# vanTeeffelenLab/ExTrack

Hardware: AMD Instinct MI355X
Metric: log-likelihood evals/sec (1e6 tracks, 2-state, len=30) (higher is better)
Workload: dtype f64

## Files before the change

### extrack_amd/csrc/xt_reg2.h

```cpp
#pragma once
#include "xt_fast2.h"
#include "xt_grad.h"


template <int F>
struct XtR2Geom {
    static constexpr int NGB = F - 1;
    static constexpr int NG = 1 << NGB;
    static constexpr int TPW = 64 / NG;
};
XT_HD constexpr int xt_r2_gbit(int F, int i) { return F == 7 ? i : (i < 2 ? i : i + 1); }
XT_HD constexpr int xt_r2_gmask(int F) { return F == 7 ? 63 : (F == 6 ? 0x3b : (F == 5 ? 0x1b : 0x0b)); }
template <int F>
XT_HD int xt_r2_slot(int lane)
{
    if (F == 7) return 0;
    int ts = (lane >> 2) & 1;
    if (F == 5) ts |= ((lane >> 5) & 1) << 1;
    if (F == 4) ts |= ((lane >> 4) & 3) << 1;
    return ts;
}

#define XT_R2_TAN0 XT_F2_TAB_BYTES
#define XT_R2_TB 36
#define XT_R2_MAXU 4
XT_HD int xt_r2_pos0(int NP) { return XT_R2_TAN0 + NP * XT_R2_TB * 8; }
XT_HD int xt_r2_acc0(int NP, int D, int KS, int tpw) { return xt_r2_pos0(NP) + XT_F2_WAVES * tpw * XT_F2_CHUNK * (D + KS) * 8; }
XT_HD int xt_r2_block_bytes(int NP, int D, int KS, int tpw) { return xt_r2_acc0(NP, D, KS, tpw) + XT_F2_WAVES * 8 * (NP + 3) * 8; }
#define XT_R2_TAB0 (XT_BLOB_HDR * 8)
#define XT_R2_GC_OFF 800
#define XT_R2_LNT_OFF 960
#define XT_R2_LNT_REL (XT_R2_LNT_OFF - XT_R2_TAB0)
static_assert(XT_R2_GC_OFF >= (XT_BLOB_HDR + XT_NTAB * 4 + 64) * 8 && XT_R2_GC_OFF + 16 <= XT_F2_NAN_OFF, "g-form constants overlap the blob / the NaN flags");
static_assert(XT_R2_LNT_OFF >= XT_F2_NAN_OFF + XT_F2_WAVES * 8 * 4 && XT_R2_LNT_OFF + 64 <= XT_F2_EXPB_OFF, "lnT' overlaps the NaN flags / the exp table");

static inline bool xt_use_reg2(int S, int NS, int F) { return S == 2 && NS == 1 && F >= 4 && F <= 7; }

template <int D, int K, int NP>
struct XtR2Lane {
    double z[2];
    int e[2];
    double m[2][D], u[2][K];
    double rz[NP ? NP : 1][2], dm[NP ? NP : 1][2][D], du[NP ? NP : 1][2][K];
};

template <int F, int D, int K, int NP, int H, bool ZF, bool LAZY, int VAR, bool FIRST = false, class Ctx>
XT_HD void xt_r2_step(Ctx& cx, char* lds, XtR2Lane<D, K, NP>& s, int tab, const double* c, const double* l2)
{
    static_assert(!FIRST || (NP == 0 && ZF && LAZY), "the merge-free first step is a step of the zero-free likelihood-only loop");
    constexpr int NGB = F - 1;
    constexpr int XB = xt_r2_gbit(F, H), PB = xt_r2_gbit(F, (H + NGB - 1) % NGB);
    const int lane = xt_opaque(cx.lane());
    const int prev = (lane >> PB) & 1;
    const int qa = Ctx::template pair_natural<XB>() ? 0 : (lane >> XB) & 1;
    const int io[2] = {(prev * 2 + qa) * 8, (prev * 2 + (qa ^ 1)) * 8};
    double TT[2], TD2[2];
    XT_UNROLL
    for (int q = 0; q < 2; ++q) {
        TT[q] = xt_at<double>(lds, tab + io[q]);
        TD2[q] = xt_at<double>(lds, XT_R2_TAB0 + 4 * 32 + io[q]);
    }

    const int e0 = s.e[0], e1 = s.e[1];
    const int emax = e0 > e1 ? e0 : e1;
    const double w0 = FIRST ? 1.0 : xt_ldexp(s.z[0], e0 - emax), w1 = FIRST ? 0.0 : xt_ldexp(s.z[1], e1 - emax);
    const double W = FIRST ? 1.0 : w0 + w1;
    double M[D], U[K];
    XT_UNROLL
    for (int d = 0; d < D; ++d) M[d] = FIRST ? s.m[0][d] : xt_fma(w1, s.m[1][d], w0 * s.m[0][d]);
    XT_UNROLL
    for (int k = 0; k < K; ++k) U[k] = FIRST ? s.u[0][k] : xt_fma(w1, s.u[1][k], w0 * s.u[0][k]);
    const bool live = ZF ? true : W > 0.0;
    const double Ws = ZF ? W : (live ? W : 1.0);
    constexpr bool RN = !LAZY || (H % XT_F2_RENORM) == 0;
    const double Wm = FIRST ? s.z[0] : (RN ? xt_frexp_mant(W) : W);
    const int We = FIRST ? e0 : (live ? (RN ? emax + xt_frexp_exp(W) : emax) : XT_EMIN);

    double Dq[2][K];
    XT_UNROLL
    for (int q = 0; q < 2; ++q)
        XT_UNROLL
        for (int k = 0; k < K; ++k) Dq[q][k] = xt_fma(Ws, l2[k] + TD2[q], U[k]);
    double rD[2][K], rW;
    if (K == 1) {
        const double d01 = Dq[0][0] * Dq[1][0];
        const double R = xt_rcp(Ws * d01);
        const double RW = R * Ws;
        rW = FIRST ? 1.0 : R * d01;
        rD[0][0] = RW * Dq[1][0];
        rD[1][0] = RW * Dq[0][0];
    } else {
        double f[2 * K + 1], pre[2 * K + 2], suf[2 * K + 2];
        f[0] = Ws;
        XT_UNROLL
        for (int q = 0; q < 2; ++q)
            XT_UNROLL
            for (int k = 0; k < K; ++k) f[1 + q * K + k] = Dq[q][k];
        pre[0] = 1.0;
        XT_UNROLL
        for (int i = 0; i < 2 * K + 1; ++i) pre[i + 1] = pre[i] * f[i];
        suf[2 * K + 1] = 1.0;
        XT_UNROLL
        for (int i = 2 * K; i >= 0; --i) suf[i] = suf[i + 1] * f[i];
        const double R = xt_rcp(pre[2 * K + 1]);
        rW = FIRST ? 1.0 : R * suf[1];
        XT_UNROLL
        for (int q = 0; q < 2; ++q)
            XT_UNROLL
            for (int k = 0; k < K; ++k) rD[q][k] = R * pre[1 + q * K + k] * suf[2 + q * K + k];
    }
    double dmW[D], dsqW = 0.0;
    XT_UNROLL
    for (int d = 0; d < D; ++d) {
        dmW[d] = xt_fma(c[d], Ws, -M[d]);
        if (K == 1) dsqW = xt_fma(dmW[d], dmW[d], dsqW);
    }
    double x[2], gf[2], tt[2][K];
    const double A = -0.5 * rW * dsqW;
    XT_UNROLL
    for (int q = 0; q < 2; ++q) {
        if (K == 1) {
            x[q] = A * rD[q][0];
            tt[q][0] = xt_fma(Ws, TD2[q], U[0]) * rD[q][0];
            gf[q] = xt_pow_half<D>(Ws * rD[q][0]);
        } else {
            double xx = 0.0, gg = 1.0;
            XT_UNROLL
            for (int d = 0; d < D; ++d) {
                xx = xt_fma(dmW[d] * dmW[d], rD[q][d], xx);
                tt[q][d] = xt_fma(Ws, TD2[q], U[d]) * rD[q][d];
                gg *= Ws * rD[q][d];
            }
            x[q] = xx * (-0.5 * rW);
            gf[q] = sqrt(gg);
        }
    }
    double p[2];
    int j[2], n[2];
    xt_exp_tab_x2(x[0], x[1], p[0], p[1], j[0], j[1], n[0], n[1]);
    double nz[2], nm[2][D], nu[2][K];
    int ne[2];
    XT_UNROLL
    for (int q = 0; q < 2; ++q) {
        int en = We + n[q];
        const double tj = xt_at<double>(lds, XT_F2_EXPB_OFF + j[q] * 8);
        double zn = (Wm * TT[q]) * (gf[q] * tj) * p[q];
        if (!LAZY) {
            en += xt_frexp_exp(zn);
            zn = xt_frexp_mant(zn);
        }
        nz[q] = zn;
        ne[q] = en > XT_EMIN ? en : XT_EMIN;
        XT_UNROLL
        for (int d = 0; d < D; ++d) nm[q][d] = xt_fma(dmW[d], tt[q][K == 1 ? 0 : d], M[d]) * rW;
        XT_UNROLL
        for (int k = 0; k < K; ++k) nu[q][k] = l2[k] * tt[q][k];
    }

    double a0 = 0.0, a1 = 0.0, cm[D], cu[K], dn[D], Aq[2][K], rq[2][K];
    if (NP > 0) {
        a0 = w0 * rW;
        a1 = w1 * rW;
        const double aa = a0 * a1;
        XT_UNROLL
        for (int d = 0; d < D; ++d) {
            cm[d] = aa * (s.m[0][d] - s.m[1][d]);
            dn[d] = dmW[d] * rW;
        }
        XT_UNROLL
        for (int k = 0; k < K; ++k) cu[k] = aa * (s.u[0][k] - s.u[1][k]);
        XT_UNROLL
        for (int q = 0; q < 2; ++q)
            XT_UNROLL
            for (int k = 0; k < K; ++k) {
                rq[q][k] = Ws * rD[q][k];
                if (K == 1)
                    Aq[q][0] = -0.5 * rq[q][0] * xt_fma(-(dsqW * rW * rW), rq[q][0], (double)D);
                else
                    Aq[q][k] = -0.5 * rq[q][k] * xt_fma(-(dn[k] * dn[k]), rq[q][k], 1.0);
            }
    }
    cx.template pair_exchange<XB>(nz[0], nz[1]);
    cx.template pair_exchange_i32<XB>(ne[0], ne[1]);
    XT_UNROLL
    for (int d = 0; d < D; ++d) cx.template pair_exchange<XB>(nm[0][d], nm[1][d]);
    XT_UNROLL
    for (int k = 0; k < K; ++k) cx.template pair_exchange<XB>(nu[0][k], nu[1][k]);
    XT_UNROLL
    for (int q = 0; q < 2; ++q) {
        s.z[q] = nz[q];
        s.e[q] = ne[q];
        XT_UNROLL
        for (int d = 0; d < D; ++d) s.m[q][d] = nm[q][d];
        XT_UNROLL
        for (int k = 0; k < K; ++k) s.u[q][k] = nu[q][k];
    }
    if (NP > 0) {
        XT_UNROLL
        for (int pp = 0; pp < NP; ++pp) {
            if (!(VAR & 1)) xt_sched_fence();
            const int tb = XT_R2_TAN0 + pp * XT_R2_TB * 8;
            double dl[K];
            XT_UNROLL
            for (int k = 0; k < K; ++k) dl[k] = xt_at<double>(lds, tb + k * 8);
            const double del = s.rz[pp][0] - s.rz[pp][1];
            const double R = xt_fma(a0, s.rz[pp][0], a1 * s.rz[pp][1]);
            double dmb[D], dub[K];
            XT_UNROLL
            for (int d = 0; d < D; ++d) dmb[d] = xt_fma(cm[d], del, xt_fma(a0, s.dm[pp][0][d], a1 * s.dm[pp][1][d]));
            XT_UNROLL
            for (int k = 0; k < K; ++k) dub[k] = xt_fma(cu[k], del, xt_fma(a0, s.du[pp][0][k], a1 * s.du[pp][1][k]));
            double hd[K];
            if (K == 1) {
                hd[0] = 0.0;
                XT_UNROLL
                for (int d = 0; d < D; ++d) hd[0] = xt_fma(dn[d], dmb[d], hd[0]);
            } else {
                XT_UNROLL
                for (int d = 0; d < D; ++d) hd[d] = dn[d] * dmb[d];
            }
            double trz[2], tdm[2][D], tdu[2][K];
            XT_UNROLL
            for (int q = 0; q < 2; ++q) {
                const double dlT = xt_at<double>(lds, tb + tab + io[q]);
                const double dd2 = xt_at<double>(lds, tb + XT_R2_TAB0 + 4 * 32 + io[q]);
                double rzn = R + dlT, dtt[K];
                XT_UNROLL
                for (int k = 0; k < K; ++k) {
                    const double ds2 = dd2 + dub[k], dden = dl[k] + ds2;
                    dtt[k] = rq[q][k] * xt_fma(-tt[q][k], dden, ds2);
                    rzn = xt_fma(Aq[q][k], dden, rzn);
                    rzn = xt_fma(rq[q][k], hd[k], rzn);
                    tdu[q][k] = xt_fma(l2[k], dtt[k], dl[k] * tt[q][k]);
                }
                trz[q] = ZF ? rzn : (live ? rzn : 0.0);
                XT_UNROLL
                for (int d = 0; d < D; ++d) {
                    const int kk = K == 1 ? 0 : d;
                    tdm[q][d] = xt_fma(dn[d], dtt[kk], xt_fma(-tt[q][kk], dmb[d], dmb[d]));
                }
            }
            cx.template pair_exchange<XB>(trz[0], trz[1]);
            XT_UNROLL
            for (int d = 0; d < D; ++d) cx.template pair_exchange<XB>(tdm[0][d], tdm[1][d]);
            XT_UNROLL
            for (int k = 0; k < K; ++k) cx.template pair_exchange<XB>(tdu[0][k], tdu[1][k]);
            XT_UNROLL
            for (int q = 0; q < 2; ++q) {
                s.rz[pp][q] = trz[q];
                XT_UNROLL
                for (int d = 0; d < D; ++d) s.dm[pp][q][d] = tdm[q][d];
                XT_UNROLL
                for (int k = 0; k < K; ++k) s.du[pp][q][k] = tdu[q][k];
            }
        }
    }
}

template <int F, int D, int H, bool FIRST = false, class Ctx>
XT_HD void xt_r2_step_g(Ctx& cx, char* lds, XtR2Lane<D, 1, 0>& s, int tab, const double* c)
{
    constexpr int NGB = F - 1;
    constexpr int XB = xt_r2_gbit(F, H), PB = xt_r2_gbit(F, (H + NGB - 1) % NGB);
    const int lane = xt_opaque(cx.lane());
    const int prev = (lane >> PB) & 1;
    const int qa = Ctx::template pair_natural<XB>() ? 0 : (lane >> XB) & 1;
    const int io[2] = {(prev * 2 + qa) * 8, (prev * 2 + (qa ^ 1)) * 8};
    double TD2[2], LT[2];
    XT_UNROLL
    for (int q = 0; q < 2; ++q) {
        TD2[q] = xt_at<double>(lds, XT_R2_TAB0 + 4 * 32 + io[q]);
        LT[q] = xt_at<double>(lds, tab + XT_R2_LNT_REL + io[q]);
    }
    const double l2 = xt_at<double>(lds, 0), nh = xt_at<double>(lds, XT_R2_GC_OFF), l22 = xt_at<double>(lds, XT_R2_GC_OFF + 8);

    const int e0 = s.e[0], e1 = s.e[1];
    const int emax = e0 > e1 ? e0 : e1;
    const double w0 = FIRST ? 1.0 : xt_ldexp(s.z[0], e0 - emax), w1 = FIRST ? 0.0 : xt_ldexp(s.z[1], e1 - emax);
    const double Ws = FIRST ? 1.0 : w0 + w1;
    double M[D];
    XT_UNROLL
    for (int d = 0; d < D; ++d) M[d] = FIRST ? s.m[0][d] : xt_fma(w1, s.m[1][d], w0 * s.m[0][d]);
    const double V = FIRST ? s.u[0][0] : xt_fma(w1, s.u[1][0], w0 * s.u[0][0]);
    constexpr bool RN = (H % XT_F2_RENORM) == 0;
    const double Wm = FIRST ? s.z[0] : (RN ? xt_frexp_mant(Ws) : Ws);
    const int We = FIRST ? e0 : (RN ? emax + xt_frexp_exp(Ws) : emax);

    const double Dq0 = xt_fma(Ws, TD2[0], V), Dq1 = xt_fma(Ws, TD2[1], V);
    const double d01 = Dq0 * Dq1;
    const double R = xt_rcp(Ws * d01);
    const double rW = FIRST ? 1.0 : R * d01;
    const double G = R * (Ws * (Ws * l2));
    const double g[2] = {G * Dq1, G * Dq0};
    double dn[D], dsq = 0.0;
    XT_UNROLL
    for (int d = 0; d < D; ++d) {
        dn[d] = xt_fma(c[d], Ws, -M[d]) * rW;
        dsq = xt_fma(dn[d], dn[d], dsq);
    }
    const double A = dsq * nh;
    double p[2];
    int j[2], n[2];
    xt_exp_tab_x2(xt_fma(A, g[0], LT[0]), xt_fma(A, g[1], LT[1]), p[0], p[1], j[0], j[1], n[0], n[1]);
    double nz[2], nm[2][D], nv[2];
    int ne[2];
    XT_UNROLL
    for (int q = 0; q < 2; ++q) {
        const int en = We + n[q];
        const double tj = xt_at<double>(lds, XT_F2_EXPB_OFF + j[q] * 8);
        nz[q] = (Wm * xt_pow_half<D>(g[q])) * (tj * p[q]);
        ne[q] = en > XT_EMIN ? en : XT_EMIN;
        XT_UNROLL
        for (int d = 0; d < D; ++d) nm[q][d] = xt_fma(-dn[d], g[q], c[d]);
        nv[q] = xt_fma(-l2, g[q], l22);
    }
    cx.template pair_exchange<XB>(nz[0], nz[1]);
    cx.template pair_exchange_i32<XB>(ne[0], ne[1]);
    XT_UNROLL
    for (int d = 0; d < D; ++d) cx.template pair_exchange<XB>(nm[0][d], nm[1][d]);
    cx.template pair_exchange<XB>(nv[0], nv[1]);
    XT_UNROLL
    for (int q = 0; q < 2; ++q) {
        s.z[q] = nz[q];
        s.e[q] = ne[q];
        XT_UNROLL
        for (int d = 0; d < D; ++d) s.m[q][d] = nm[q][d];
        s.u[q][0] = nv[q];
    }
}

template <int F, class Ctx>
XT_HD double xt_r2_gsum(Ctx& cx, double v)
{
    constexpr int NGB = F - 1;
    v += cx.template xor_f64<xt_r2_gbit(F, 0)>(v);
    v += cx.template xor_f64<xt_r2_gbit(F, 1)>(v);
    v += cx.template xor_f64<xt_r2_gbit(F, 2)>(v);
    if (NGB > 3) v += cx.template xor_f64<xt_r2_gbit(F, NGB > 3 ? 3 : 0)>(v);
    if (NGB > 4) v += cx.template xor_f64<xt_r2_gbit(F, NGB > 4 ? 4 : 0)>(v);
    if (NGB > 5) v += cx.template xor_f64<xt_r2_gbit(F, NGB > 5 ? 5 : 0)>(v);
    return v;
}
template <int F, class Ctx>
XT_HD int xt_r2_gmax(Ctx& cx, int v)
{
    constexpr int NGB = F - 1;
    auto mx = [](int a, int b) XT_INL { return a > b ? a : b; };
    v = mx(v, cx.template xor_i32<xt_r2_gbit(F, 0)>(v));
    v = mx(v, cx.template xor_i32<xt_r2_gbit(F, 1)>(v));
    v = mx(v, cx.template xor_i32<xt_r2_gbit(F, 2)>(v));
    if (NGB > 3) v = mx(v, cx.template xor_i32<xt_r2_gbit(F, NGB > 3 ? 3 : 0)>(v));
    if (NGB > 4) v = mx(v, cx.template xor_i32<xt_r2_gbit(F, NGB > 4 ? 4 : 0)>(v));
    if (NGB > 5) v = mx(v, cx.template xor_i32<xt_r2_gbit(F, NGB > 5 ? 5 : 0)>(v));
    return v;
}

template <int F, int D, int K, int NP, class Ctx, class GetPos>
XT_HD void xt_r2_chain(Ctx& cx, char* lds, XtR2Lane<D, K, NP>& s, int T, int stay_from, GetPos& getpos)
{
    constexpr int NGB = F - 1;
    const int lane = xt_opaque(cx.lane());
    double z = s.z[0];
    int e = s.e[0];
    XT_UNROLL
    for (int t = 1; t < NGB; ++t) {
        if (t > T) break;
        const int prev = (lane >> xt_r2_gbit(F, t == 1 ? NGB - 1 : t - 2)) & 1;
        const int q = (lane >> xt_r2_gbit(F, t - 1)) & 1;
        const int io = (prev * 2 + q) * 8;
        const double TT = xt_at<double>(lds, XT_R2_TAB0 + (t >= stay_from ? 32 : 0) + io);
        const double d2 = xt_at<double>(lds, XT_R2_TAB0 + 4 * 32 + io);
        double c[D], l2[K];
        getpos(t, c, l2);
        double tt[K], r[K], dm[D], x = 0.0, gf;
        XT_UNROLL
        for (int k = 0; k < K; ++k) {
            const double a = d2 + s.u[0][k];
            r[k] = xt_rcp(l2[k] + a);
            tt[k] = a * r[k];
        }
        XT_UNROLL
        for (int d = 0; d < D; ++d) dm[d] = c[d] - s.m[0][d];
        if (K == 1) {
            XT_UNROLL
            for (int d = 0; d < D; ++d) x = xt_fma(dm[d], dm[d], x);
            x *= -0.5 * r[0];
            gf = xt_pow_half<D>(r[0]);
        } else {
            double gg = 1.0;
            XT_UNROLL
            for (int d = 0; d < D; ++d) {
                x = xt_fma(-0.5 * dm[d] * dm[d], r[d], x);
                gg *= r[d];
            }
            gf = sqrt(gg);
        }
        double p;
        int j, n;
        xt_exp_tab_x1(x, p, j, n);
        z = (z * TT) * (gf * xt_at<double>(lds, XT_F2_EXPB_OFF + j * 8)) * p;
        e += n;
        XT_UNROLL
        for (int d = 0; d < D; ++d) s.m[0][d] = xt_fma(dm[d], tt[K == 1 ? 0 : d], s.m[0][d]);
        XT_UNROLL
        for (int k = 0; k < K; ++k) s.u[0][k] = l2[k] * tt[k];
    }
    int dummy = 0;
    XT_UNROLL
    for (int i = 0; i < NGB - 1; ++i)
        if (i >= T) dummy |= 1 << xt_r2_gbit(F, i);
    const bool live = (lane & dummy) == 0;
    s.z[0] = live ? xt_frexp_mant(z) : 0.0;
    s.e[0] = live ? e + xt_frexp_exp(z) : XT_EMIN;
}

template <int F, int D, int K, int NP, int VAR = 0, class Ctx>
XT_HD void xt_r2_body(const XtKernelArgs& a, const XtGradArgs& ga, Ctx& cx)
{
    int lb, nb;
    const XtBucketDesc b = xt_bind_bucket(a, cx.block(), cx.nblocks(), lb, nb);
    typedef XtR2Geom<F> Gm;
    constexpr int NGB = Gm::NGB, TPW = Gm::TPW;
    constexpr int GMASK = xt_r2_gmask(F);
    const int lane = cx.lane();
    const int wib = cx.wave_in_block();
    const int nwb = cx.waves_per_block();
    const int L = b.L;
    const int KS = a.locerr_mode ? a.KS : 0;
    double* smem = cx.smem();
    char* lds = (char*)smem;

    const int ntab = xt_tab_doubles(2, 2);
    for (int i = cx.tid(); i < ntab; i += cx.nthreads()) smem[i] = xt_blob_ptr(a)[i];
    if (NP > 0)
        for (int i = cx.tid(); i < NP * XT_R2_TB; i += cx.nthreads()) xt_at<double>(lds, XT_R2_TAN0 + i * 8) = ga.dblob[i];
    const int NU = NP > 0 ? ga.NU : 0, NPT = NP + NU;
    for (int i = cx.tid(); i < NU * XT_R2_TB; i += cx.nthreads()) xt_at<double>(lds, XT_R2_TAN0 + (NP * XT_R2_TB + i) * 8) = ga.udblob[i];
    cx.sync();
    xt_f2_check_lds_base(lds);
    xt_f2_build_exp_table(cx, lds, XT_F2_EXPB_OFF, (const double*)(lds + XT_F2_T64_OFF));
    const bool gform = NP == 0 && K == 1 && a.well_scaled == 2 && a.locerr_mode == 0;
    if constexpr (NP == 0 && K == 1) {
        if (gform && cx.tid() < 10) {
            const int i = cx.tid();
            const double l2 = smem[0];
            if (i < 8)
                xt_at<double>(lds, XT_R2_LNT_OFF + i * 8) = log(smem[XT_BLOB_HDR + i]) - 0.5 * D * log(l2);
            else
                xt_at<double>(lds, XT_R2_GC_OFF + (i - 8) * 8) = i == 8 ? -0.5 / l2 : 2.0 * l2;
        }
    }
    cx.sync();
    const double* hdr = smem;

    const int ts = xt_r2_slot<F>(lane);
    const bool leader = (lane & GMASK) == 0;
    const int tlast = L - 1;
    const int stay_from = a.min_len > 2 ? a.min_len : 2;
    const int vfin = (b.isBL ? 2 : 0) + (tlast >= stay_from ? 1 : 0);
    double l2g[K];
    XT_UNROLL
    for (int k = 0; k < K; ++k) l2g[k] = hdr[k];
    const bool well_scaled = a.well_scaled != 0;
    const bool chain = NP == 0 && well_scaled;

    double* pos = (double*)(lds + xt_r2_pos0(NPT)) + wib * TPW * XT_F2_CHUNK * (D + KS);
    double* sig = pos + TPW * XT_F2_CHUNK * D;
    double* accp = (double*)(lds + xt_r2_acc0(NPT, D, KS, TPW)) + (wib * 8 + ts) * (NPT + 3);
    if (leader) {
        if (NP == 0) {
            accp[0] = 1.0;
            accp[1] = 0.0;
            accp[2] = 0.0;
        } else {
            for (int i = 0; i < NPT + 1; ++i) accp[i] = 0.0;
        }
    }

    const int64_t nbatch = (b.N + TPW - 1) / TPW;
    const int64_t W0 = (int64_t)lb * nwb + wib, NW = (int64_t)nb * nwb;
    for (int64_t batch = W0; batch < nbatch; batch += NW) {
        const int64_t trk = batch * TPW + ts;
        const bool act = trk < b.N;

        auto stage = [&](int p0) XT_INL {
            cx.wave_sync();
            for (int i = lane; i < TPW * XT_F2_CHUNK * D; i += 64) {
                const int t_ = i / (XT_F2_CHUNK * D), r = i - t_ * (XT_F2_CHUNK * D);
                const int64_t tk = batch * TPW + t_;
                const int64_t tkc = tk < b.N ? tk : b.N - 1;
                const int pp = p0 + r / D;
                if (pp < L) {
                    const double v = b.tracks[(tkc * L + p0) * D + r];
                    pos[i] = v;
                    if (v != v) xt_at<int>(lds, XT_F2_NAN_OFF + (wib * 8 + t_) * 4) = 1;
                }
            }
            if (KS)
                for (int i = lane; i < TPW * XT_F2_CHUNK * KS; i += 64) {
                    const int t_ = i / (XT_F2_CHUNK * KS), r = i - t_ * (XT_F2_CHUNK * KS);
                    const int64_t tk = batch * TPW + t_;
                    const int64_t tkc = tk < b.N ? tk : b.N - 1;
                    const int pp = p0 + r / KS;
                    if (pp < L) {
                        const double v = b.sigma[(tkc * L + p0) * KS + r];
                        sig[i] = v;
                        if (v != v) xt_at<int>(lds, XT_F2_NAN_OFF + (wib * 8 + t_) * 4) = 1;
                    }
                }
            cx.wave_sync();
        };
        auto getpos = [&](int t, double* c, double* l2) XT_INL {
            const int r = t & (XT_F2_CHUNK - 1);
            XT_UNROLL
            for (int d = 0; d < D; ++d) c[d] = pos[(ts * XT_F2_CHUNK + r) * D + d];
            if (KS == 0) {
                XT_UNROLL
                for (int k = 0; k < K; ++k) l2[k] = xt_at<double>(lds, k * 8);
            } else {
                XT_UNROLL
                for (int k = 0; k < K; ++k) {
                    double sg = sig[(ts * XT_F2_CHUNK + r) * KS + (KS == 1 ? 0 : k)];
                    if (a.locerr_mode == 2) {
                        sg = xt_fma(sg, hdr[3], hdr[4]);
                        sg = sg < 1e-6 ? 1e-6 : sg;
                    }
                    l2[k] = sg * sg;
                }
            }
        };

        XtR2Lane<D, K, NP> s;
#define XT_R2_PHASE(H, ZF_, LAZY_)                                                                     \
    if (NGB > (H) && t <= tend2 && ph == (H)) {                                                        \
        double c[D], l2[K];                                                                            \
        getpos(t, c, l2);                                                                              \
        xt_r2_step<F, D, K, NP, ((H) < NGB ? (H) : 0), ZF_, LAZY_, VAR>(cx, lds, s, XT_R2_TABSEL, c, l2);   \
        ++t;                                                                                           \
        ph = (H) + 1 == NGB ? 0 : (H) + 1;                                                             \
    }
#define XT_R2_PHASE_G(H)                                                                               \
    if (NGB > (H) && t <= tend2 && ph == (H)) {                                                        \
        double c[D], l2[K];                                                                            \
        getpos(t, c, l2);                                                                              \
        xt_r2_step_g<F, D, ((H) < NGB ? (H) : 0)>(cx, lds, s, XT_R2_TABSEL, c);                        \
        ++t;                                                                                           \
        ph = (H) + 1 == NGB ? 0 : (H) + 1;                                                             \
    }
#define XT_R2_PHASES(ZF_, LAZY_) \
    XT_R2_PHASE(0, ZF_, LAZY_)   \
    XT_R2_PHASE(1, ZF_, LAZY_)   \
    XT_R2_PHASE(2, ZF_, LAZY_)   \
    XT_R2_PHASE(3, ZF_, LAZY_)   \
    XT_R2_PHASE(4, ZF_, LAZY_)   \
    XT_R2_PHASE(5, ZF_, LAZY_)
#define XT_R2_TABSEL tab
        auto run_steps = [&](int& t, int tend, int tab) XT_INL {
            int ph = (t - 1) % NGB;
            const int tend2 = tend;
            if (!well_scaled) {
                while (t <= tend2) { XT_R2_PHASES(false, false) }
                return;
            }
            if constexpr (NP == 0 && K == 1) {
                if (gform) {
                    while (t <= tend2) {
                        XT_R2_PHASE_G(0)
                        XT_R2_PHASE_G(1)
                        XT_R2_PHASE_G(2)
                        XT_R2_PHASE_G(3)
                        XT_R2_PHASE_G(4)
                        XT_R2_PHASE_G(5)
                    }
                    return;
                }
            }
            while (t <= tend2) { XT_R2_PHASES(true, true) }
        };
#undef XT_R2_TABSEL
#define XT_R2_TABSEL (XT_R2_TAB0 + (t >= stay_from ? 32 : 0))
        auto run_steps_g = [&](int& t, int tend) XT_INL {
            int ph = (t - 1) % NGB;
            const int tend2 = tend;
            if (well_scaled) {
                while (t <= tend2) { XT_R2_PHASES(false, true) }
            } else {
                while (t <= tend2) { XT_R2_PHASES(false, false) }
            }
        };
#undef XT_R2_TABSEL
#undef XT_R2_PHASES
#undef XT_R2_PHASE_G
#undef XT_R2_PHASE

        XtAcc tot;
        tot.clear();
        double gacc[NP ? NP : 1];
        double uacc[XT_R2_MAXU];
        int fe = XT_EMIN;
        int t = 1;
        if (lane < 8) xt_at<int>(lds, XT_F2_NAN_OFF + (wib * 8 + lane) * 4) = 0;
        for (int p0 = 0; p0 < L; p0 += XT_F2_CHUNK) {
            stage(p0);
            if (p0 == 0) {
                constexpr int NBIT = xt_r2_gbit(F, NGB - 1);
                double c0[D], l20[K];
                getpos(0, c0, l20);
                const bool live0 = chain || (lane & (GMASK & ~(1 << NBIT))) == 0;
                const int s0 = (lane >> NBIT) & 1;
                s.z[0] = live0 ? hdr[8 + s0] : 0.0;
                s.e[0] = live0 ? 0 : XT_EMIN;
                s.z[1] = 0.0;
                s.e[1] = XT_EMIN;
                XT_UNROLL
                for (int q = 0; q < 2; ++q) {
                    XT_UNROLL
                    for (int d = 0; d < D; ++d) s.m[q][d] = c0[d];
                    XT_UNROLL
                    for (int k = 0; k < K; ++k) s.u[q][k] = l20[k];
                }
                XT_UNROLL
                for (int pp = 0; pp < NP; ++pp) {
                    const int tb = XT_R2_TAN0 + pp * XT_R2_TB * 8;
                    s.rz[pp][0] = live0 ? xt_at<double>(lds, tb + (8 + s0) * 8) : 0.0;
                    s.rz[pp][1] = 0.0;
                    XT_UNROLL
                    for (int q = 0; q < 2; ++q) {
                        XT_UNROLL
                        for (int d = 0; d < D; ++d) s.dm[pp][q][d] = 0.0;
                        XT_UNROLL
                        for (int k = 0; k < K; ++k) s.du[pp][q][k] = xt_at<double>(lds, tb + k * 8);
                    }
                }
                if constexpr (NP == 0) {
                    if (chain) {
                        const int T = L - 2 < NGB - 1 ? L - 2 : NGB - 1;
                        xt_r2_chain<F>(cx, lds, s, T, stay_from, getpos);
                        if (L - 2 >= F - 1) {
                            double c[D], l2[K];
                            getpos(F - 1, c, l2);
                            bool first_done = false;
                            if constexpr (K == 1) {
                                if (gform) {
                                    s.u[0][0] += l2[0];
                                    xt_r2_step_g<F, D, NGB - 1, true>(cx, lds, s, XT_R2_TAB0 + (F - 1 >= stay_from ? 32 : 0), c);
                                    first_done = true;
                                }
                            }
                            if (!first_done) xt_r2_step<F, D, K, NP, NGB - 1, true, true, VAR, true>(cx, lds, s, XT_R2_TAB0 + (F - 1 >= stay_from ? 32 : 0), c, l2);
                            t = F;
                        } else {
                            t = L - 1 > 1 ? L - 1 : 1;
                        }
                    }
                }
            }
            const int tend = (L - 2 < p0 + XT_F2_CHUNK - 1) ? L - 2 : p0 + XT_F2_CHUNK - 1;
            if (NP == 0) {
                run_steps(t, tend < stay_from - 1 ? tend : stay_from - 1, XT_R2_TAB0);
                run_steps(t, tend, XT_R2_TAB0 + 32);
            } else {
                run_steps_g(t, tend);
            }
            if (tlast < p0 || tlast >= p0 + XT_F2_CHUNK) continue;
            double cl[D], l2l[K];
            getpos(tlast, cl, l2l);
            if constexpr (NP == 0 && K == 1) {
                if (gform && L - 2 >= F - 1) l2l[0] = 0.0;
            }
            const int hp = (tlast - 2 + NGB) % NGB;
            const int pbit = (F == 7 || hp < 2) ? hp : hp + 1;
            const int prev = (lane >> pbit) & 1;
            double wm[4], rr[4][K], dq[2][D], dsqQ[2];
            int we[4];
            XT_UNROLL
            for (int Q = 0; Q < 2; ++Q) {
                dsqQ[Q] = 0.0;
                XT_UNROLL
                for (int d = 0; d < D; ++d) {
                    dq[Q][d] = cl[d] - s.m[Q][d];
                    dsqQ[Q] = xt_fma(dq[Q][d], dq[Q][d], dsqQ[Q]);
                }
                double x[2], gf[2];
                XT_UNROLL
                for (int q = 0; q < 2; ++q) {
                    const double d2 = xt_at<double>(lds, XT_R2_TAB0 + 4 * 32 + (prev * 2 + q) * 8);
                    if (K == 1) {
                        const double r = xt_rcp(d2 + s.u[Q][0] + l2l[0]);
                        rr[Q * 2 + q][0] = r;
                        x[q] = -0.5 * dsqQ[Q] * r;
                        gf[q] = xt_pow_half<D>(r);
                    } else {
                        double xx = 0.0, gg = 1.0;
                        XT_UNROLL
                        for (int d = 0; d < D; ++d) {
                            const double r = xt_rcp(d2 + s.u[Q][d] + l2l[d]);
                            rr[Q * 2 + q][d] = r;
                            xx = xt_fma(-0.5 * dq[Q][d] * dq[Q][d], r, xx);
                            gg *= r;
                        }
                        x[q] = xx;
                        gf[q] = sqrt(gg);
                    }
                }
                double p[2];
                int j[2], n[2];
                xt_exp_tab_x2(x[0], x[1], p[0], p[1], j[0], j[1], n[0], n[1]);
                XT_UNROLL
                for (int q = 0; q < 2; ++q) {
                    const double tf = xt_at<double>(lds, XT_R2_TAB0 + vfin * 32 + (prev * 2 + q) * 8);
                    wm[Q * 2 + q] = s.z[Q] * tf * gf[q] * xt_at<double>(lds, XT_F2_EXPB_OFF + j[q] * 8) * p[q];
                    we[Q * 2 + q] = s.e[Q] + n[q];
                    tot.add(wm[Q * 2 + q], we[Q * 2 + q]);
                }
            }
            fe = xt_r2_gmax<F>(cx, tot.m != 0.0 ? tot.e : XT_EMIN);
            if (NP > 0) {
                double ws[4];
                XT_UNROLL
                for (int i = 0; i < 4; ++i) ws[i] = wm[i] != 0.0 ? xt_ldexp(wm[i], we[i] - fe) : 0.0;
                XT_UNROLL
                for (int pp = 0; pp < NP; ++pp) {
                    const int tb = XT_R2_TAN0 + pp * XT_R2_TB * 8;
                    double dl[K];
                    XT_UNROLL
                    for (int k = 0; k < K; ++k) dl[k] = xt_at<double>(lds, tb + k * 8);
                    double acc = 0.0;
                    XT_UNROLL
                    for (int Q = 0; Q < 2; ++Q) {
                        XT_UNROLL
                        for (int q = 0; q < 2; ++q) {
                            const double dlT = xt_at<double>(lds, tb + XT_R2_TAB0 + vfin * 32 + (prev * 2 + q) * 8);
                            const double dd2 = xt_at<double>(lds, tb + XT_R2_TAB0 + 4 * 32 + (prev * 2 + q) * 8);
                            double rel = s.rz[pp][Q] + dlT;
                            if (K == 1) {
                                const double r = rr[Q * 2 + q][0];
                                const double dden = dd2 + s.du[pp][Q][0] + dl[0];
                                double ddsq = 0.0;
                                XT_UNROLL
                                for (int d = 0; d < D; ++d) ddsq = xt_fma(-2.0 * dq[Q][d], s.dm[pp][Q][d], ddsq);
                                rel -= 0.5 * r * (D * dden + ddsq - dsqQ[Q] * r * dden);
                            } else {
                                XT_UNROLL
                                for (int d = 0; d < D; ++d) {
                                    const double r = rr[Q * 2 + q][d];
                                    const double dden = dd2 + s.du[pp][Q][d] + dl[d];
                                    rel -= 0.5 * r * (dden - 2.0 * dq[Q][d] * s.dm[pp][Q][d] - dq[Q][d] * dq[Q][d] * r * dden);
                                }
                            }
                            acc = xt_fma(ws[Q * 2 + q], ws[Q * 2 + q] != 0.0 ? rel : 0.0, acc);
                        }
                    }
                    gacc[pp] = acc;
                }
                XT_UNROLL
                for (int u = 0; u < XT_R2_MAXU; ++u) {
                    double acc = 0.0;
                    if (u < NU) {
                        const int tb = XT_R2_TAN0 + (NP + u) * XT_R2_TB * 8;
                        XT_UNROLL
                        for (int i = 0; i < 4; ++i) acc = xt_fma(ws[i], xt_at<double>(lds, tb + XT_R2_TAB0 + vfin * 32 + (prev * 2 + (i & 1)) * 8), acc);
                    }
                    uacc[u] = acc;
                }
            }
        }
        double sum = xt_r2_gsum<F>(cx, tot.m != 0.0 ? xt_ldexp(tot.m, tot.e - fe) : 0.0);
        const bool poisoned = xt_at<int>(lds, XT_F2_NAN_OFF + (wib * 8 + ts) * 4) != 0;
        if (poisoned) sum = NAN;
        if (NP == 0) {
            if (act && leader) {
                if (b.ll_out) b.ll_out[trk] = log(sum) + (double)fe * XT_LN2 + b.ll_const;
                const double pm = accp[0] * xt_frexp_mant(sum);
                double acce = accp[1] + (double)(fe + xt_frexp_exp(sum) + xt_frexp_exp(pm));
                if (sum == 0.0) acce = -INFINITY;
                accp[0] = xt_frexp_mant(pm);
                accp[1] = acce;
                accp[2] += 1.0;
            }
        } else {
            const double rs = 1.0 / sum;
            double gsum[NP ? NP : 1];
            XT_UNROLL
            for (int pp = 0; pp < NP; ++pp) gsum[pp] = xt_r2_gsum<F>(cx, gacc[pp]);
            double usum[XT_R2_MAXU];
            XT_UNROLL
            for (int u = 0; u < XT_R2_MAXU; ++u) usum[u] = u < NU ? xt_r2_gsum<F>(cx, uacc[u]) : 0.0;
            if (act && leader) {
                const double ll = log(sum) + (double)fe * XT_LN2 + b.ll_const;
                if (b.ll_out) b.ll_out[trk] = ll;
                accp[0] += ll;
                XT_UNROLL
                for (int pp = 0; pp < NP; ++pp) accp[1 + pp] += gsum[pp] * rs;
                const int nsteps = L - 2 > 0 ? L - 2 : 0;
                const int n1 = nsteps >= stay_from ? nsteps - stay_from + 1 : 0, n0 = nsteps - n1;
                XT_UNROLL
                for (int u = 0; u < XT_R2_MAXU; ++u)
                    if (u < NU) {
                        const int tb = XT_R2_TAN0 + (NP + u) * XT_R2_TB * 8;
                        const double rzu = xt_at<double>(lds, tb + 8 * 8) + n0 * xt_at<double>(lds, tb + XT_R2_TAB0) + n1 * xt_at<double>(lds, tb + XT_R2_TAB0 + 32);
                        accp[1 + NP + u] += usum[u] * rs + rzu;
                    }
            }
        }
        cx.wave_sync();
    }

    cx.sync();
    if (NP == 0) {
        if (leader) smem[wib * TPW + ts] = accp[2] > 0.0 ? log(accp[0]) + accp[1] * XT_LN2 + accp[2] * b.ll_const : 0.0;
        cx.sync();
        if (cx.tid() == 0) {
            double sacc = 0.0;
            for (int i = 0; i < nwb * TPW; ++i) sacc += smem[i];
            a.partials[cx.block()] = sacc;
        }
    } else {
        const double* acc0 = (const double*)(lds + xt_r2_acc0(NPT, D, KS, TPW));
        for (int col = cx.tid(); col < NPT + 1; col += cx.nthreads()) {
            double sacc = 0.0;
            for (int w = 0; w < nwb; ++w)
                for (int i = 0; i < TPW; ++i) sacc += acc0[(w * 8 + i) * (NPT + 3) + col];
            ga.gpartials[(int64_t)cx.block() * (NPT + 1) + col] = sacc;
        }
    }
}
```

Measured before the change: 416.3.

## Track g-form weights in log domain with periodic LDS atomic rebase

Replaces the per-lane integer exponent bookkeeping (ldexp alignment, exp-table evaluation of new weights, int exchange) in the 2-state g-form step with a log-domain offset carried per lane. The pair weights are combined via a single exp of their log difference. Once per cycle the group subtracts an integer shift, agreed through an LDS atomic max, and records that shift per thread in LDS so the final log-likelihood can be corrected. It also moves the NP==0 accumulators into LDS slots indexed per track. The intent is to cut exp-table work and exchanges in the hot step. The cost is extra LDS atomics, wave syncs and possible precision or overflow risk in the log offset.

```diff
diff --git a/extrack_amd/csrc/xt_reg2.h b/extrack_amd/csrc/xt_reg2.h
--- a/extrack_amd/csrc/xt_reg2.h
+++ b/extrack_amd/csrc/xt_reg2.h
@@ -26,7 +26,12 @@
 #define XT_R2_MAXU 4
 XT_HD int xt_r2_pos0(int NP) { return XT_R2_TAN0 + NP * XT_R2_TB * 8; }
 XT_HD int xt_r2_acc0(int NP, int D, int KS, int tpw) { return xt_r2_pos0(NP) + XT_F2_WAVES * tpw * XT_F2_CHUNK * (D + KS) * 8; }
-XT_HD int xt_r2_block_bytes(int NP, int D, int KS, int tpw) { return xt_r2_acc0(NP, D, KS, tpw) + XT_F2_WAVES * 8 * (NP + 3) * 8; }
+#define XT_R2_RC_ARR (XT_F2_WAVES * 64 * 8)
+XT_HD int xt_r2_rc0(int D, int KS, int tpw) { return xt_r2_acc0(0, D, KS, tpw) + XT_F2_WAVES * 8 * 3 * 8; }
+XT_HD int xt_r2_block_bytes(int NP, int D, int KS, int tpw)
+{
+    return xt_r2_acc0(NP, D, KS, tpw) + XT_F2_WAVES * 8 * (NP + 3) * 8 + (NP == 0 ? 2 * XT_R2_RC_ARR + XT_F2_WAVES * 8 * 8 : 0);
+}
 #define XT_R2_TAB0 (XT_BLOB_HDR * 8)
 #define XT_R2_GC_OFF 800
 #define XT_R2_LNT_OFF 960
@@ -257,8 +262,12 @@
     }
 }
 
+#ifndef XT_R2_RC_H
+#define XT_R2_RC_H 0
+#endif
+#define XT_R2_RC_NONE (-2147483647 - 1)
 template <int F, int D, int H, bool FIRST = false, class Ctx>
-XT_HD void xt_r2_step_g(Ctx& cx, char* lds, XtR2Lane<D, 1, 0>& s, int tab, const double* c)
+XT_HD void xt_r2_step_g(Ctx& cx, char* lds, XtR2Lane<D, 1, 0>& s, double (&lx)[2], int tab, const double* c)
 {
     constexpr int NGB = F - 1;
     constexpr int XB = xt_r2_gbit(F, H), PB = xt_r2_gbit(F, (H + NGB - 1) % NGB);
@@ -274,17 +283,37 @@
     }
     const double l2 = xt_at<double>(lds, 0), nh = xt_at<double>(lds, XT_R2_GC_OFF), l22 = xt_at<double>(lds, XT_R2_GC_OFF + 8);
 
-    const int e0 = s.e[0], e1 = s.e[1];
-    const int emax = e0 > e1 ? e0 : e1;
-    const double w0 = FIRST ? 1.0 : xt_ldexp(s.z[0], e0 - emax), w1 = FIRST ? 0.0 : xt_ldexp(s.z[1], e1 - emax);
+    double w0 = 1.0, w1 = 0.0, base = lx[0];
+    if (!FIRST) {
+        const double dl = lx[1] - lx[0];
+        double p;
+        int j, n;
+        xt_exp_tab_x1(-fabs(dl), p, j, n);
+        const double E = xt_ldexp(xt_at<double>(lds, XT_F2_EXPB_OFF + j * 8) * p, n);
+        const bool up = dl > 0.0;
+        w0 = s.z[0] * (up ? E : 1.0);
+        w1 = s.z[1] * (up ? 1.0 : E);
+        base = up ? lx[1] : lx[0];
+    }
     const double Ws = FIRST ? 1.0 : w0 + w1;
     double M[D];
     XT_UNROLL
     for (int d = 0; d < D; ++d) M[d] = FIRST ? s.m[0][d] : xt_fma(w1, s.m[1][d], w0 * s.m[0][d]);
     const double V = FIRST ? s.u[0][0] : xt_fma(w1, s.u[1][0], w0 * s.u[0][0]);
-    constexpr bool RN = (H % XT_F2_RENORM) == 0;
+    constexpr bool RN = !FIRST && (H % XT_F2_RENORM) == 0;
     const double Wm = FIRST ? s.z[0] : (RN ? xt_frexp_mant(Ws) : Ws);
-    const int We = FIRST ? e0 : (RN ? emax + xt_frexp_exp(Ws) : emax);
+    if (RN) base = xt_fma((double)xt_frexp_exp(Ws), XT_LN2, base);
+    if (!FIRST && H == XT_R2_RC_H) {
+        const int tid = xt_opaque(cx.tid());
+        const int rc0 = xt_r2_rc0(D, 0, XtR2Geom<F>::TPW);
+        const int cell = rc0 + (tid & ~xt_r2_gmask(F)) * 8;
+        cx.atomic_max_i32(&xt_at<int>(lds, cell), (int)fmin(fmax(base, -1e9), 1e9));
+        cx.wave_sync();
+        const int sh = xt_at<int>(lds, cell);
+        base -= (double)sh;
+        xt_at<unsigned int>(lds, rc0 + XT_R2_RC_ARR + tid * 8) += (unsigned int)sh;
+    }
+    if (!FIRST && H == (XT_R2_RC_H + 1) % NGB) xt_at<int>(lds, xt_r2_rc0(D, 0, XtR2Geom<F>::TPW) + (xt_opaque(cx.tid()) & ~xt_r2_gmask(F)) * 8) = XT_R2_RC_NONE;
 
     const double Dq0 = xt_fma(Ws, TD2[0], V), Dq1 = xt_fma(Ws, TD2[1], V);
     const double d01 = Dq0 * Dq1;
@@ -299,30 +328,24 @@
         dsq = xt_fma(dn[d], dn[d], dsq);
     }
     const double A = dsq * nh;
-    double p[2];
-    int j[2], n[2];
-    xt_exp_tab_x2(xt_fma(A, g[0], LT[0]), xt_fma(A, g[1], LT[1]), p[0], p[1], j[0], j[1], n[0], n[1]);
-    double nz[2], nm[2][D], nv[2];
-    int ne[2];
+    double ny[2], nl[2], nm[2][D], nv[2];
     XT_UNROLL
     for (int q = 0; q < 2; ++q) {
-        const int en = We + n[q];
-        const double tj = xt_at<double>(lds, XT_F2_EXPB_OFF + j[q] * 8);
-        nz[q] = (Wm * xt_pow_half<D>(g[q])) * (tj * p[q]);
-        ne[q] = en > XT_EMIN ? en : XT_EMIN;
+        ny[q] = Wm * xt_pow_half<D>(g[q]);
+        nl[q] = xt_fma(A, g[q], LT[q]) + base;
         XT_UNROLL
         for (int d = 0; d < D; ++d) nm[q][d] = xt_fma(-dn[d], g[q], c[d]);
         nv[q] = xt_fma(-l2, g[q], l22);
     }
-    cx.template pair_exchange<XB>(nz[0], nz[1]);
-    cx.template pair_exchange_i32<XB>(ne[0], ne[1]);
+    cx.template pair_exchange<XB>(ny[0], ny[1]);
+    cx.template pair_exchange<XB>(nl[0], nl[1]);
     XT_UNROLL
     for (int d = 0; d < D; ++d) cx.template pair_exchange<XB>(nm[0][d], nm[1][d]);
     cx.template pair_exchange<XB>(nv[0], nv[1]);
     XT_UNROLL
     for (int q = 0; q < 2; ++q) {
-        s.z[q] = nz[q];
-        s.e[q] = ne[q];
+        s.z[q] = ny[q];
+        lx[q] = nl[q];
         XT_UNROLL
         for (int d = 0; d < D; ++d) s.m[q][d] = nm[q][d];
         s.u[q][0] = nv[q];
@@ -423,7 +446,7 @@
     constexpr int NGB = Gm::NGB, TPW = Gm::TPW;
     constexpr int GMASK = xt_r2_gmask(F);
     const int lane = cx.lane();
-    const int wib = cx.wave_in_block();
+    const int wib = NP == 0 ? cx.uniform(cx.wave_in_block()) : cx.wave_in_block();
     const int nwb = cx.waves_per_block();
     const int L = b.L;
     const int KS = a.locerr_mode ? a.KS : 0;
@@ -467,11 +490,16 @@
     double* pos = (double*)(lds + xt_r2_pos0(NPT)) + wib * TPW * XT_F2_CHUNK * (D + KS);
     double* sig = pos + TPW * XT_F2_CHUNK * D;
     double* accp = (double*)(lds + xt_r2_acc0(NPT, D, KS, TPW)) + (wib * 8 + ts) * (NPT + 3);
+    auto accb = [&]() XT_INL { return xt_r2_acc0(0, D, KS, TPW) + (wib * 8 + xt_r2_slot<F>(xt_opaque(cx.lane()))) * 24; };
+    auto rcacc = [&]() XT_INL { return xt_r2_rc0(D, KS, TPW) + XT_R2_RC_ARR + xt_opaque(cx.tid()) * 8; };
+    auto rcsum = [&]() XT_INL { return xt_r2_rc0(D, KS, TPW) + 2 * XT_R2_RC_ARR + (wib * 8 + xt_r2_slot<F>(xt_opaque(cx.lane()))) * 8; };
     if (leader) {
         if (NP == 0) {
-            accp[0] = 1.0;
-            accp[1] = 0.0;
-            accp[2] = 0.0;
+            const int ab = accb();
+            xt_at<double>(lds, ab) = 1.0;
+            xt_at<double>(lds, ab + 8) = 0.0;
+            xt_at<double>(lds, ab + 16) = 0.0;
+            xt_at<double>(lds, rcsum()) = 0.0;
         } else {
             for (int i = 0; i < NPT + 1; ++i) accp[i] = 0.0;
         }
@@ -531,6 +559,7 @@
         };
 
         XtR2Lane<D, K, NP> s;
+        double lx[2] = {0.0, 0.0};
 #define XT_R2_PHASE(H, ZF_, LAZY_)                                                                     \
     if (NGB > (H) && t <= tend2 && ph == (H)) {                                                        \
         double c[D], l2[K];                                                                            \
@@ -543,7 +572,7 @@
     if (NGB > (H) && t <= tend2 && ph == (H)) {                                                        \
         double c[D], l2[K];                                                                            \
         getpos(t, c, l2);                                                                              \
-        xt_r2_step_g<F, D, ((H) < NGB ? (H) : 0)>(cx, lds, s, XT_R2_TABSEL, c);                        \
+        xt_r2_step_g<F, D, ((H) < NGB ? (H) : 0)>(cx, lds, s, lx, XT_R2_TABSEL, c);                        \
         ++t;                                                                                           \
         ph = (H) + 1 == NGB ? 0 : (H) + 1;                                                             \
     }
@@ -600,6 +629,10 @@
         int fe = XT_EMIN;
         int t = 1;
         if (lane < 8) xt_at<int>(lds, XT_F2_NAN_OFF + (wib * 8 + lane) * 4) = 0;
+        if (NP == 0) {
+            xt_at<int>(lds, rcacc()) = 0;
+            xt_at<int>(lds, rcacc() - XT_R2_RC_ARR) = XT_R2_RC_NONE;
+        }
         for (int p0 = 0; p0 < L; p0 += XT_F2_CHUNK) {
             stage(p0);
             if (p0 == 0) {
@@ -643,7 +676,9 @@
                             if constexpr (K == 1) {
                                 if (gform) {
                                     s.u[0][0] += l2[0];
-                                    xt_r2_step_g<F, D, NGB - 1, true>(cx, lds, s, XT_R2_TAB0 + (F - 1 >= stay_from ? 32 : 0), c);
+                                    lx[0] = (double)s.e[0] * XT_LN2;
+                                    xt_r2_step_g<F, D, NGB - 1, true>(cx, lds, s, lx, XT_R2_TAB0 + (F - 1 >= stay_from ? 32 : 0), c);
+                                    s.e[0] = s.e[1] = 0;
                                     first_done = true;
                                 }
                             }
@@ -689,6 +724,7 @@
                         const double r = xt_rcp(d2 + s.u[Q][0] + l2l[0]);
                         rr[Q * 2 + q][0] = r;
                         x[q] = -0.5 * dsqQ[Q] * r;
+                        if constexpr (NP == 0) x[q] += lx[Q];
                         gf[q] = xt_pow_half<D>(r);
                     } else {
                         double xx = 0.0, gg = 1.0;
@@ -769,14 +805,19 @@
         const bool poisoned = xt_at<int>(lds, XT_F2_NAN_OFF + (wib * 8 + ts) * 4) != 0;
         if (poisoned) sum = NAN;
         if (NP == 0) {
-            if (act && leader) {
-                if (b.ll_out) b.ll_out[trk] = log(sum) + (double)fe * XT_LN2 + b.ll_const;
-                const double pm = accp[0] * xt_frexp_mant(sum);
-                double acce = accp[1] + (double)(fe + xt_frexp_exp(sum) + xt_frexp_exp(pm));
+            const int lz = xt_opaque(cx.lane());
+            const int64_t trk = batch * TPW + xt_r2_slot<F>(lz);
+            if (trk < b.N && (lz & GMASK) == 0) {
+                const double rcs = (double)xt_at<int>(lds, rcacc());
+                if (b.ll_out) b.ll_out[trk] = log(sum) + (double)fe * XT_LN2 + b.ll_const + rcs;
+                xt_at<double>(lds, rcsum()) += rcs;
+                const int ab = accb();
+                const double pm = xt_at<double>(lds, ab) * xt_frexp_mant(sum);
+                double acce = xt_at<double>(lds, ab + 8) + (double)(fe + xt_frexp_exp(sum) + xt_frexp_exp(pm));
                 if (sum == 0.0) acce = -INFINITY;
-                accp[0] = xt_frexp_mant(pm);
-                accp[1] = acce;
-                accp[2] += 1.0;
+                xt_at<double>(lds, ab) = xt_frexp_mant(pm);
+                xt_at<double>(lds, ab + 8) = acce;
+                xt_at<double>(lds, ab + 16) += 1.0;
             }
         } else {
             const double rs = 1.0 / sum;
@@ -808,7 +849,10 @@
 
     cx.sync();
     if (NP == 0) {
-        if (leader) smem[wib * TPW + ts] = accp[2] > 0.0 ? log(accp[0]) + accp[1] * XT_LN2 + accp[2] * b.ll_const : 0.0;
+        if (leader) {
+            const double* ac = &xt_at<double>(lds, accb());
+            smem[wib * TPW + ts] = ac[2] > 0.0 ? log(ac[0]) + ac[1] * XT_LN2 + ac[2] * b.ll_const + xt_at<double>(lds, rcsum()) : 0.0;
+        }
         cx.sync();
         if (cx.tid() == 0) {
             double sacc = 0.0;
```

After: 433.1, median of 6. 1.04x the previous value.
